# dleeim/Safe-Bayesian-Optimization

Hardware: AMD Instinct MI355X
Metric: candidate-points/sec, SafeOpt posterior+safe-set sweep (higher is better)
Workload: dtype f64

## Files before the change

include/safebo.h:

```cpp
#ifndef SAFEBO_H
#define SAFEBO_H

#include <stdint.h>

#ifdef __cplusplus
extern "C" {
#endif

#define SBO_ABI_VERSION 3
#define SBO_MAX_D 8
#define SBO_MAX_Q 8
#define SBO_MAX_N 2048

enum sbo_status {
  SBO_OK = 0,
  SBO_E_INVALID = -1,
  SBO_E_NOMEM = -2,
  SBO_E_HIP = -3,
  SBO_E_NO_MODEL = -4,
  SBO_E_NO_CANDIDATES = -5,
  SBO_E_EMPTY_SAFE_SET = -6,
  SBO_E_COMM = -7,
  SBO_E_UNSUPPORTED = -8
};
// ... 98 lines not shown
  double total_ms;
  double posterior_flops;
  int64_t candidates;
  int32_t posterior_launches;
  int32_t posterior_kernel;
  double posterior_executed_flops;
  double posterior_setup_ms;
  int64_t fp64_rechecks;
  double recheck_ms;
  double set_phase_ms;
  int32_t host_syncs;
  int32_t comm_calls;
  int64_t comm_bytes;
  double guard_dm[SBO_MAX_Q], guard_dv[SBO_MAX_Q], guard_rl[SBO_MAX_Q];
  double guard_ms;
  int32_t halo_reruns;
  int32_t set_path;
  int64_t guard_audit_samples, guard_audit_violations;
  double guard_audit_worst;
  double guard_analytic_dm[SBO_MAX_Q], guard_analytic_dv[SBO_MAX_Q], guard_probe_dm[SBO_MAX_Q], guard_probe_dv[SBO_MAX_Q];
  int64_t k1_tiles_skipped;
  int64_t k1_tiles_skipped_safe;
  int64_t k1_tiles_resident_c, k1_tiles_resident_o;
  int64_t guard_audit_skipped;
  double list_index_build_ms;
  int64_t list_index_leaf_pairs, list_index_nodes_skipped;
  double fp32_band_dm[SBO_MAX_Q], fp32_band_dv[SBO_MAX_Q];
} sbo_profile;

int sbo_version(void);
const char* sbo_last_error(void);
int sbo_device_count(int* count);
int sbo_init(int device_id, sbo_ctx** out);
int sbo_shutdown(sbo_ctx* ctx);
int sbo_synchronize(sbo_ctx* ctx);

#define SBO_COMM_ID_BYTES 128
int sbo_comm_unique_id(void* id_out );
int sbo_comm_init(sbo_ctx* ctx, int world_size, int rank, const void* id);
int sbo_comm_barrier(sbo_ctx* ctx);
typedef int (*sbo_relay_allreduce_fn)(void* user, void* buf, int64_t count, int elem, int op);
typedef int (*sbo_relay_allgather_fn)(void* user, const void* send, void* recv, int64_t bytes_per_rank);
int sbo_comm_init_relay(sbo_ctx* ctx, int world_size, int rank, sbo_relay_allreduce_fn allreduce,
                        sbo_relay_allgather_fn allgather, void* user);

int sbo_model_set(sbo_ctx* ctx, int dtype, const char* kernel, int n, int d, int q,
// ... 323 lines not shown
```

safe-bayesian-optimization_amd/_lib.py:

```python
from __future__ import annotations

import ctypes as C
import os

SBO_MAX_D = 8
SBO_MAX_Q = 8
SBO_MAX_N = 2048
SBO_COMM_ID_BYTES = 128
SBO_ROBUST_MAX_SCEN = 8
SBO_MAX_BATCH = 64
SBO_MAX_APPEND = 64
SBO_EXPANDER_MAX_POINTS = 65536
SBO_EXPANDER_MAX_SCRATCH = 1 << 32
SBO_MAX_PATHS = 64
SBO_MAX_FEATURES = 8192
SBO_PATHS_MAX_POINTS = 1 << 24
SBO_PATHS_MAX_VALUES = 1 << 32
SBO_REFINE_PATHS_MAX_STARTS = 64
SBO_JOINT_MAX_POINTS = 2048

SBO_F64, SBO_F32 = 0, 1
SBO_MEAN, SBO_UCB, SBO_LCB, SBO_VAR = 0, 1, 2, 3
SBO_MASK_S, SBO_MASK_U, SBO_MASK_M, SBO_MASK_G, SBO_MASK_O = 0, 1, 2, 3, 4

# ... 157 lines not shown
class JointOpts(C.Structure):
    _fields_ = [("output", C.c_int32), ("n_draws", C.c_int32), ("noise", C.c_int32), ("maximize", C.c_int32), ("jitter", C.c_double)]


class JointResult(C.Structure):
    _fields_ = [("index", C.c_int64 * SBO_MAX_PATHS), ("value", C.c_double * SBO_MAX_PATHS), ("pivot_min", C.c_double),
                ("pivot_row", C.c_int64)]


class Profile(C.Structure):
    _fields_ = [
        ("posterior_ms", C.c_double), ("classify_ms", C.c_double), ("expander_ms", C.c_double),
        ("argreduce_ms", C.c_double), ("comm_ms", C.c_double), ("total_ms", C.c_double),
        ("posterior_flops", C.c_double), ("candidates", C.c_int64), ("posterior_launches", C.c_int32),
        ("posterior_kernel", C.c_int32), ("posterior_executed_flops", C.c_double), ("posterior_setup_ms", C.c_double),
        ("fp64_rechecks", C.c_int64), ("recheck_ms", C.c_double),
        ("set_phase_ms", C.c_double), ("host_syncs", C.c_int32), ("comm_calls", C.c_int32), ("comm_bytes", C.c_int64),
        ("guard_dm", C.c_double * SBO_MAX_Q), ("guard_dv", C.c_double * SBO_MAX_Q), ("guard_rl", C.c_double * SBO_MAX_Q),
        ("guard_ms", C.c_double), ("halo_reruns", C.c_int32), ("set_path", C.c_int32),
        ("guard_audit_samples", C.c_int64), ("guard_audit_violations", C.c_int64), ("guard_audit_worst", C.c_double),
        ("guard_analytic_dm", C.c_double * SBO_MAX_Q), ("guard_analytic_dv", C.c_double * SBO_MAX_Q),
        ("guard_probe_dm", C.c_double * SBO_MAX_Q), ("guard_probe_dv", C.c_double * SBO_MAX_Q),
        ("k1_tiles_skipped", C.c_int64), ("k1_tiles_skipped_safe", C.c_int64),
        ("k1_tiles_resident_c", C.c_int64), ("k1_tiles_resident_o", C.c_int64), ("guard_audit_skipped", C.c_int64),
        ("list_index_build_ms", C.c_double), ("list_index_leaf_pairs", C.c_int64), ("list_index_nodes_skipped", C.c_int64),
        ("fp32_band_dm", C.c_double * SBO_MAX_Q), ("fp32_band_dv", C.c_double * SBO_MAX_Q),
    ]


RELAY_ALLREDUCE = C.CFUNCTYPE(C.c_int, C.c_void_p, C.c_void_p, C.c_int64, C.c_int, C.c_int)
RELAY_ALLGATHER = C.CFUNCTYPE(C.c_int, C.c_void_p, C.c_void_p, C.c_void_p, C.c_int64)

_P = C.c_void_p
_DP = C.POINTER(C.c_double)
SYMBOLS = [
    ("sbo_version", C.c_int, []),
    ("sbo_last_error", C.c_char_p, []),
    ("sbo_device_count", C.c_int, [C.POINTER(C.c_int)]),
    ("sbo_init", C.c_int, [C.c_int, C.POINTER(_P)]),
    ("sbo_shutdown", C.c_int, [_P]),
    ("sbo_synchronize", C.c_int, [_P]),
    ("sbo_comm_unique_id", C.c_int, [_P]),
    ("sbo_comm_init", C.c_int, [_P, C.c_int, C.c_int, _P]),
    ("sbo_comm_barrier", C.c_int, [_P]),
    ("sbo_comm_init_relay", C.c_int, [_P, C.c_int, C.c_int, RELAY_ALLREDUCE, RELAY_ALLGATHER, _P]),
    ("sbo_model_set", C.c_int, [_P, C.c_int, C.c_char_p, C.c_int, C.c_int, C.c_int, _P, _P, _P, _P, _P, _P, _P, _P]),
    ("sbo_model_set_list", C.c_int, [_P, C.c_int, C.c_char_p, C.c_int, C.c_int, C.c_int, _P, _P, _P, _P, _P, _P, _P, _P]),
# ... 92 lines not shown
```

safe-bayesian-optimization_amd/csrc/api.hip:

```cpp
#include <algorithm>
#include <cmath>
#include <cstring>
#include <limits>
#include <memory>
#include <chrono>
#include "internal.hpp"
#include "device_common.hpp"

namespace sbo {

static thread_local std::string g_err;

int fail(int code, const std::string& msg) {
  g_err = msg;
  return code;
}
int hip_fail(hipError_t e, const char* what) {
  g_err = std::string("HIP: ") + hipGetErrorString(e) + " in " + what;
  return SBO_E_HIP;
}
int ensure(DevBuf& b, size_t bytes) {
  if (bytes == 0) bytes = 16;
  if (b.bytes >= bytes) return SBO_OK;
  b.reset();
// ... 232 lines not shown
#define OPT_SCALED(key, field, scale, lo, hi, msg, effect, hook) {key, nullptr, &Options::field, kTakeScaled, msg, lo, hi, 0, scale, effect, hook}
const OptRow kOptions[] = {
    OPT_BOOL(halo_spec, kOptNothing, hook_halo),
    OPT_BOOL(comm_events, kOptNothing, nullptr),
    OPT_SCALED("cheb_tol_e17", cheb_tol, 1e-17, 0, 0, nullptr, kOptPlans, nullptr),
    OPT_RANGE(tensor_guess_pct, 10, 400, "tensor_guess_pct must be within 10 .. 400", kOptTensor, hook_tensor_guess),
    OPT_BOOL(tensor_cheb, kOptTensor, nullptr),
    OPT_CLAMP(exact_lazy, 0, 2, 1, kOptNothing, nullptr),
    OPT_BOOL(chol_async, kOptNothing, nullptr),
    OPT_RANGE(bilinear, 0, 2, "bilinear must be 0 (off), 1 (on; a model's first sweep by node interpolation) or 2 (on, K1b's plan from the first sweep)", kOptPlans, nullptr),
    OPT_BOOL(phase_events, kOptNothing, nullptr),
    OPT_RAW(scan_waves, kOptNothing, nullptr),
    OPT_BOOL(set_lanes, kOptNothing, nullptr),
    OPT_BOOL(result_mirror, kOptNothing, nullptr),
    OPT_BOOL(set_fuse, kOptNothing, nullptr),
    OPT_RANGE(col_path, 0, 2, "col_path must be 0 (never), 1 (auto) or 2 (whenever the grid's shape allows)", kOptNothing, nullptr),
    OPT_RANGE(guard_audit, 0, 1 << 20, "guard_audit: samples per sweep, 0 (off) .. 1048576", kOptNothing, hook_audit),
    OPT_SCALED("guard_audit_scale_ppm", audit_scale, 1e-6, 1, 1000000000, "guard_audit_scale_ppm: 1 .. 1e9", kOptNothing, hook_audit_scale),
    OPT_RANGE(guard_audit_every, 1, 1 << 20, "guard_audit_every: 1 .. 1048576 sweeps", kOptNothing, hook_audit_every),
    OPT_RANGE(grad_defer, 0, 3, "grad_defer must be 0 .. 3", kOptInterp, nullptr),
    OPT_BOOL(k1_sched, kOptNothing, nullptr),
    OPT_BOOL(k1_resident, kOptNothing, nullptr),
    OPT_BOOL(k1_skip_safe, kOptNothing, nullptr),
    OPT_BOOL(col_overlap, kOptNothing, nullptr),
    OPT_RANGE(col_queue, 64, 128, "col_queue must be within 64 .. 128 (the default)", kOptNothing, nullptr),
    OPT_BOOL(scan_blocks, kOptNothing, nullptr),
    OPT_RANGE(fuse_classify, -1, 1, "fuse_classify must be -1 (auto), 0 or 1", kOptNothing, nullptr),
    OPT_BOOL(goose_pairs, kOptNothing, nullptr),
    OPT_RANGE(guard_band, 0, 2, "guard_band must be 0 (off), 1 (on) or 2 (re-evaluate on every sweep)", kOptPlansBand, nullptr),
    OPT_BOOL(fp64_recheck, kOptNothing, nullptr),
    OPT_BOOL(comm_selftest, kOptNothing, hook_selftest),
    OPT_RANGE(refine_lds, 0, 1, "refine_lds must be 0 (stream M) or 1 (LDS when it fits)", kOptNothing, nullptr),
    OPT_RANGE(lipschitz_lds, 0, 1, "lipschitz_lds must be 0 (stream X_norm and alpha) or 1 (LDS when they fit)", kOptNothing, nullptr),
    OPT_RANGE(list_index, -1, 1, "list_index must be -1 (auto), 0 (never) or 1 (always)", kOptNothing, nullptr),
    OPT_RANGE(posterior_path, 0, 2, "posterior_path must be 0 (auto), 1 (generic) or 2 (generic, chunked)", kOptPosterior, nullptr),
};
#undef OPT_BOOL
#undef OPT_RANGE
#undef OPT_CLAMP
#undef OPT_RAW
#undef OPT_SCALED
}

int sbo_set_option(sbo_ctx* c, const char* key, int64_t value) {
  if (!c || !key) return fail(SBO_E_INVALID, "ctx/key is NULL");
  for (const OptRow& r : kOptions) {
// ... 494 lines not shown
```

safe-bayesian-optimization_amd/csrc/bilinear_post.inc.hpp:

```cpp


constexpr int kFuseRow = 4 + 2 * kMaxQ;
constexpr int kFuseVmin = 4, kFuseRmax = 4 + kMaxQ;
struct PostCtx {
  double* lds;
  int tid, lane, wave, rb0, cs0, nrb, ncs;
  int st_rb, st_cs, st_off, a_lo, b_st, a_rd;
  unsigned int ucnt0;
  long long nlines;
  bool full;
  bool imode;
  const double* var_rd;
  uint8_t *S, *U;
  double bconf, bb;
  int cS, cU;
  double rmax;
  LcbBand lband;
  bool gb_on;
  double vminS;
  int cB;
  int role;
  unsigned int bw[8];
  unsigned int* lds_bits;
  double umin;
// ... 1013 lines not shown
  const double gmax = ROLE == 1 ? lrec[ctile] : 0.0;
  post_partials<4>(sh, cx.lane, cx.wave, gmax, ROLE == 1, cx.cS, cx.cU, ROLE == 2 ? -cx.umin : cx.rmax, cx.cB, cx.vminS,
                   Lpart + ((size_t)o * tgy + by) * tgx + bx, cpart + (ROLE == 2 ? ntile : (size_t)0) + ctile, pcap, ROLE == 2, px.cb.slots,
                   (int)(ctile & (kColSlots - 1)), o, ROLE == 1 ? (int)by : -1, (int)bx, cx.xmin, false);
  if (ROLE == 1 && cx.tid < 128) {
    unsigned long long sw = 0ull, uw = 0ull;
#pragma unroll
    for (int w = 0; w < 4; ++w) {
      const unsigned int pc = bits[w * 128 + cx.tid];
      sw |= (unsigned long long)(pc & 0xffffu) << (16 * w);
      uw |= (unsigned long long)(pc >> 16) << (16 * w);
    }
    const size_t col = (size_t)cx.cs0 * 16u + cx.tid;
    px.cb.Sw[(size_t)by * cx.ucnt0 + col] = sw;
    px.cb.Uw[(size_t)by * cx.ucnt0 + col] = uw;
    if (uw != 0ull) atomicOr(&px.cb.Usum[col], 1ull << by);
  }
#ifdef SBO_PHASE_CLOCKS
  __syncthreads();
  if (threadIdx.x == 0) wg_trace_row(o, clk_in_, clk_ld_, wall_clock64(), (unsigned int)ctile, 4u);
#endif
}


__global__ __launch_bounds__(256, 3) void k_bgrad(const ModelConst mc, const CandSpec cs, const double* __restrict__ VA, size_t sVA,
                                                  const double* __restrict__ P0f, int KB, int nrb, int ncs, long long nlines, int gx, int gy,
                                                  const int* __restrict__ eff, const double* __restrict__ gtmax,
                                                  const unsigned long long* __restrict__ gkey, const double* __restrict__ xn0, int q,
                                                  double* __restrict__ Lpart, unsigned long long* __restrict__ slots,
                                                  int o_first ) {
  extern __shared__ double lds[];
  PostCtx cx;
  cx.lds = lds;
  cx.tid = threadIdx.x; cx.lane = cx.tid & 63; cx.wave = cx.tid >> 6;
  cx.nrb = nrb; cx.ncs = ncs;
  cx.ucnt0 = (unsigned int)cs.count[0];
  cx.nlines = nlines;
  cx.imode = true;
  const int st_i = cx.tid >> 5, st_j = cx.tid & 31;
  cx.st_off = st_j * 8;
  cx.a_lo = st_i < 4 ? st_i * 256 + (st_j >> 3) * 64 + (st_j & 7) * 4 : -1;
  cx.b_st = 1024 + st_i * 256 + cx.st_off;
  cx.a_rd = (((cx.lane >> 4) << 2) + (cx.lane & 3)) * 2;
  cx.var_rd = nullptr; cx.S = nullptr; cx.U = nullptr;
  cx.bconf = 0.0; cx.bb = 0.0; cx.cS = cx.cU = cx.cB = 0; cx.rmax = -1.0;
  cx.lband = LcbBand{0.0, 0.0}; cx.gb_on = false; cx.vminS = 1e300;
// ... 229 lines not shown
  SBO_HIP(hipFuncSetAttribute(reinterpret_cast<const void*>(k_bgrad), hipFuncAttributeMaxDynamicSharedMemorySize, (int)L.lds));
  hipLaunchKernelGGL(k_bgrad, dim3((unsigned)std::min<long long>((long long)L.rows_out, 2ll * c->n_cu)), dim3(256), L.lds, gs, c->mc, c->cs, g.VA,
                     g.sVA, g.P0f, g.KB0, g.nrb, g.ncs0, L.nlines, (int)L.gx, (int)L.gy, (const int*)g.eff, g.gtmax, g.gkey,
                     (const double*)c->bl_small.p, L.q, L.lrows, L.colw ? L.px.cb.slots : (unsigned long long*)nullptr, (L.req.sweep_lean && L.q >= 2) ? 1 : 0);
  SBO_HIP(hipEventRecord(c->ev_grad[2], gs));
  c->grad_pending = true;
  L.px.nograd = 1;
  return SBO_OK;
}

static void gemm_post_part(GemmLaunch& L, int part) {
  sbo_ctx* c = L.c;
  const GemmOps& g = L.g;
  const CandSpec& cs = c->cs;
  const bool colw = L.colw, fuse = L.fuse;
  const int q = L.q;
  const ColPartRows& rows = L.out.col_rows;
  PostExtra& px = L.px;
  px.o0 = colw ? 1 - part : 0;
  const bool last = !colw || part == 1;
  const decltype(&k_bpost<1, 0>) kposts[3] = {k_bpost<1, 0>, k_bpost<1, 1>, k_bpost<1, 2>};
  const auto kpost = kposts[colw ? 1 + part : 0];
  px.tlist = nullptr;
  if (L.sched_l1 && part == 0 && px.encl) {
    hipLaunchKernelGGL(k_bl_sched_tiles1, dim3((L.gx * L.gy + kSchedWaves - 1) / kSchedWaves), dim3(64 * kSchedWaves), 0, c->stream, c->mc, (const double*)px.encl, (int)(L.gx * L.gy), (int)L.gx,
                       (int)L.gy, (unsigned int)L.cnt0, L.req.fuse_b, L.gb_fused, g.gtmax, g.gkey, q, px.skip, L.sched_l1, L.sched_cap1, px.cb.Sw, px.cb.Uw,
                       px.cb.Usum, px.cb.slots, L.lrows, rows.base, rows.cap, px.skip_safe, L.res_rows ? (const double*)L.lrec : (const double*)nullptr,
                       L.res_c ? 1 : 0);
    px.tlist = L.sched_l1;
    px.tshift = kTlistShift;
    px.tcap = L.sched_cap1;
  }
  if (L.sched_l2 && part == 1) {
    hipLaunchKernelGGL(k_bl_sched_list2, dim3(1), dim3(1024), 0, c->stream, rows.base, rows.cap, (int)(L.gx * L.gy), L.sched_l2,
                       L.lrows, L.sched_l1, L.res_o ? (const uint8_t*)L.omap : (const uint8_t*)nullptr, px.cb.slots);
    px.tlist = L.sched_l2;
    px.tshift = 0;
    px.tcap = (int)(L.gx * L.gy);
    L.out.col_sched = true;
  }
  px.tgx = (int)L.gx;
  px.tgy = (int)L.gy;
  const dim3 grid = px.tlist ? dim3((unsigned)px.tcap << px.tshift) : dim3(L.gx, L.gy, (unsigned)(colw ? 1 : q));
  px.front_only = 0;
  const bool light_c = L.res_c && part == 0 && px.tlist != nullptr, light_o = L.res_o && part == 1 && px.tlist != nullptr;
  if (light_c) {
    hipExtLaunchKernelGGL(k_bres<1>, grid, dim3(256), 0, c->stream, nullptr, c->col.ev[0], 0, cs, (const double*)c->mean.p, (const double*)c->var.p,
                          L.lrows, L.req.fuse_b, (unsigned long long*)c->cpart.p, c->cpart_cap, L.gb_fused, (const double*)L.lrec, px);
  }
  if (light_o) {
    hipLaunchKernelGGL(k_bres<2>, grid, dim3(256), 0, c->stream, cs, (const double*)c->mean.p, (const double*)c->var.p, L.lrows, L.req.fuse_b,
                       (unsigned long long*)c->cpart.p, c->cpart_cap, (const GuardBand*)nullptr, (const double*)nullptr, px);
    px.front_only = 1;
  }
  if (!light_c) {
    hipExtLaunchKernelGGL(kpost, grid, dim3(256), L.lds, c->stream, nullptr,
                          (L.req.lmax_defer && last) ? c->ev[1] : ((colw && part == 0) ? c->col.ev[0] : nullptr), 0,
                          c->mc, cs, g.BtA, g.sBtA, g.P0f, g.sP0f, g.VA, g.sVA, g.SBf, g.sSBf, g.KB0, g.KS0, g.KBm, g.KSm, g.KBm2, g.nrb, g.ncs0,
                          L.nlines, (double*)c->mean.p, (double*)c->var.p, L.defer ? L.lrows + (size_t)L.rows_out * q : L.lrows,
                          (const double*)c->bl_small.p , fuse ? (uint8_t*)(q > 2 ? c->fuseS.p : c->maskS.p) : (uint8_t*)nullptr,
                          fuse ? (uint8_t*)(q > 2 ? c->fuseU.p : c->maskU.p) : (uint8_t*)nullptr, L.req.fuse_b, (unsigned long long*)c->cpart.p,
                          c->cpart_cap, L.gb_fused, (const int*)g.eff, g.gtmax, g.gkey, g.imode, px);
  }
  if (colw && part == 0 && L.record_encl) {
    hipLaunchKernelGGL(k_bl_enclose, dim3(L.gx, L.gy), dim3(128), 0, c->stream, (const double*)c->mean.p + (size_t)cs.n_local,
                       (const double*)c->var.p + (size_t)cs.n_local, L.cnt0, L.encl, (const double*)L.lrows + L.ntiles, L.lrec);
    c->bl.encl_ready = true;
    c->bl.lrows_ready = L.lrec != nullptr;
  }
  if (colw && part == 0 && !L.interp && c->bl.encl_ready && !px.encl) c->bl.vals_ready = true;
}

static void gemm_flops(const GemmLaunch& L) {
  sbo_ctx* c = L.c;
  const GemmOps& g = L.g;
  const int q = L.q;
  const double tiles2 = (double)g.nrb * g.ncs0;
  if (L.interp) {
// ... 68 lines not shown
```

safe-bayesian-optimization_amd/csrc/internal.hpp:

```cpp
#pragma once
#include <hip/hip_runtime.h>
#include <stddef.h>
#include <stdint.h>
#include <cmath>
#include <string>
#include <type_traits>
#include <vector>
#include "../../include/safebo.h"

namespace sbo {

constexpr int kGuardRefMaxNpad = 1008;
constexpr int kMaxD = SBO_MAX_D;
constexpr int kMaxQ = SBO_MAX_Q;

struct RcScal {
  unsigned long long ulo_key, uhi_key, vmax_key;
  long long count;
};
struct RcHead {
  RcScal sc;
  unsigned long long deferred;
  unsigned long long lmin_key;
  unsigned long long all_ranks;
// ... 108 lines not shown
  long long n = 0;
  int d = 0;
  int perm_half = 0;
  DevBuf box;
  DevBuf keys, vals, hist;
  DevBuf xs;
  DevBuf stats;
  Event ev0, ev1;
};

struct ColBits {
  unsigned long long* Sw;
  unsigned long long* Uw;
  unsigned long long* Usum;
  unsigned long long* slots;
};
constexpr int kColSlots = 64;
enum ColSlotField { kSlotUmin = 0 , kSlotS, kSlotU, kSlotB , kSlotVmin0, kSlotVmin1 ,
                    kSlotRmax1 , kSlotL0, kSlotL1 ,
                    kSlotRowMask ,
                    kSlotSkip ,
                    kSlotSkipSafe ,
                    kSlotResC, kSlotResO ,
                    kColSlotFields };
__host__ __device__ inline bool col_slot_is_min(int f) { return f == kSlotUmin || f == kSlotVmin0 || f == kSlotVmin1; }
constexpr unsigned int kTlistUnsafe = 0x80000000u, kTlistSafe = 0x40000000u;
constexpr unsigned char kSkipUnsafe = 1, kSkipSafe = 2;
constexpr int kTlistShift = 5, kTlistShards = 1 << kTlistShift, kTlistHead = 32;
struct PostExtra {
  int o0;
  int q;
  int lean;
  long long fstride;
  int nograd;
  ColBits cb;
  const double* encl;
  uint8_t* skip;
  int skip_safe;
  const unsigned int* tlist;
  int tshift, tcap;
  int tgx, tgy;
  int front_only;
  uint8_t* omap;
};

struct GemmOps {
// ... 216 lines not shown
  hipStream_t stream2 = nullptr;
  hipStream_t stream_audit = nullptr;
  hipStream_t stream4 = nullptr;
  hipStream_t stream3 = nullptr;
  int n_cu = 256;
  int decide_wg_per_cu = 1;
  struct Options {
    int chol_async = 1;
    int exact_lazy = 1;
    double cheb_tol = 4e-15;
    int tensor_cheb = 1;
    int tensor_guess_pct = 100;
    int guard_band = 1;
    int guard_audit = 1024;
    int guard_audit_every = 16;
    double audit_scale = 1.0;
    int set_lanes = 1;
    int refine_lds = 1;
    int lipschitz_lds = 1;
    int list_index = -1;
    int k1_sched = 1;
    int k1_resident = 1;
    int k1_skip_safe = 1;
    int comm_events = 0;
    int col_path = 1;
    int col_overlap = 1;
    int col_queue = 128;
    int grad_defer = 1;
    int halo_spec = 1;
    int scan_waves = 1;
    int scan_blocks = 1;
    int result_mirror = 1;
    int set_fuse = 1;
    int fuse_classify = -1;
    int goose_pairs = 0;
    int phase_events = 0;
    int bilinear = 1;
    int posterior_path = 0;
    int fp64_recheck = 1;
    int comm_selftest = 0;
  } opt;
  bool has_model = false;
  int dtype = SBO_F64;
  sbo::ModelConst mc{};
  sbo::DevBuf Fpk;
  sbo::DevBuf As;
// ... 285 lines not shown
```

safe-bayesian-optimization_amd/csrc/sets.hip:

```cpp
#include <algorithm>
#include <cstdio>
#include <cstdlib>
#include <cmath>
#include <cstring>
#include <type_traits>
#include <hip/hip_ext.h>
#include "device_common.hpp"

namespace sbo {

int comm_allreduce_max_u64(sbo_ctx* c, unsigned long long* dev, int count);
int comm_allreduce_min_u64(sbo_ctx* c, unsigned long long* dev, int count);
int comm_allreduce_sum_f64(sbo_ctx* c, double* dev, int count);
int comm_allgather_bytes(sbo_ctx* c, const void* send, void* recv, size_t bytes_per_rank);

constexpr double kInfD = 1.0e300;
constexpr int kArgSlots = 16;

struct SweepScalars {
  unsigned long long ustar_key;
  unsigned long long rmax_key[kMaxQ];
  long long count_S, count_U, count_M;
  long long count_set[kMaxQ];
  long long n_amb, n_amb_total;
  long long n_scan;
  long long halo_short;
  double arg_val[kArgSlots];
  long long arg_idx[kArgSlots];
  double arg_d[kArgSlots];
  long long n_guard;
  long long guard_slot[kArgSlots];
  long long tiles_skipped;
  long long tiles_skipped_safe;
  long long tiles_resident_c, tiles_resident_o;
  unsigned long long ticket;
  long long n_guard_cls;
  long long guard_nb0;
  unsigned long long vmin_key[kMaxQ];
  double gb_du[kMaxQ];
  double gb_rl[kMaxQ];
  double arg_e1[kArgSlots], arg_e2[kArgSlots];
  long long arg_ei[kArgSlots];
};
constexpr size_t kScalHost = offsetof(SweepScalars, ticket);
static_assert(sizeof(SweepScalars) <= sizeof(ScalBlock::scalars) && sizeof(SweepScalars) <= sizeof(PinnedBack::scalars), "SweepScalars fits its region of the scalar block and of the pinned block");

struct Best {
  double v;
  long long i;
  double d;
  double e1, e2;
  long long ei;
};
template <bool MAX>
__host__ __device__ __forceinline__ Best best_none() { return Best{0.0, -1, 0.0, MAX ? -kInfD : kInfD, MAX ? -kInfD : kInfD, -1}; }

template <bool MAX>
// ... 1898 lines not shown
  hipExtLaunchKernelGGL(k_sweep_finals<true>, dim3((unsigned)q), dim3(256), 0, c->stream, nullptr, mirrored ? c->ev[4] : nullptr, 0,
                        (const unsigned char*)pbase, pstride, n > 0 ? nb : 0, sc,
                        lanes ? (const SweepScalars*)c->lane[1].scal.p : (const SweepScalars*)nullptr,
                        mirrored ? (unsigned char*)c->h_back : (unsigned char*)nullptr, c->Lmax, gb_of<T>(c, v) ? 1 : 0);
  SBO_HIP(hipGetLastError());
  if ((rc = sweep_exchange_back(c, h, AllMax().v, Lk, c->ev[4], mirrored))) return rc;
  if (lazy_exact && (h.n_amb > 0 || c->opt.exact_lazy == 2) && (rc = late_exact_pass<T>(c, o, v, nb, h, Lk, launch_exact_d<T>))) return rc;
  if (multi_rank(c)) {
    sbo_sweep_opts o2 = *o;
    SetView v2 = v;
    if (halo_rerun(c, h, Lk, o2, v2)) return sweep_safeopt_t<T>(c, &o2, v2, res);
  }
  }
  c->masks_valid = true;
  c->last_sweep = 1;
  if (getenv("SBO_DEBUG_SCAN")) fprintf(stderr, "[safebo] open candidates scanned (last constraint) %lld, exact rechecks %lld\n", h.n_scan, h.n_amb_total);

  if ((rc = sweep_profile(c, kSafeOpt, reuse))) return rc;
  c->prof.set_path = colpath ? 1 : 0;
  c->prof.k1_tiles_skipped = colpath ? h.tiles_skipped : 0;
  c->prof.k1_tiles_skipped_safe = colpath ? h.tiles_skipped_safe : 0;
  c->prof.k1_tiles_resident_c = colpath ? h.tiles_resident_c : 0;
  c->prof.k1_tiles_resident_o = colpath ? h.tiles_resident_o : 0;
  if (colpath && !reuse)
    c->last_k1_flops = std::max(0.0, c->last_k1_flops - (double)h.tiles_resident_c * c->last_k1_tile_flops[1] - (double)h.tiles_resident_o * c->last_k1_tile_flops[0]);

  memset(res, 0, sizeof(*res));
  res->count_S = h.count_S;
  res->count_U = h.count_U;
  res->count_M = h.count_M;
  res->n_exact_rechecks = h.n_amb_total;
  res->guard_band = h.n_guard;
  c->gb.first = h.n_guard;
  for (int i = 0; i < q; ++i) memcpy(&res->L[i], &Lk[i], 8);
  if (o->lean && q >= 2) res->L[0] = 0.0;
  res->minimizer_index = -1;
  res->expander_index = -1;
  for (int cc = 1; cc <= kMaxQ; ++cc) res->expander_index_c[cc - 1] = -1;
  if (h.count_S == 0) return fail(SBO_E_EMPTY_SAFE_SET, "safe set S_t is empty on this candidate set");
  res->u_star = ord_val(h.ustar_key);
  res->minimizer_index = h.arg_idx[0];
  res->minimizer_std = std::sqrt(h.arg_val[0]);
  coords_of(c, res->minimizer_index, res->minimizer_x);
  double best_std = 0.0;
  int best_c = 0;
  for (int cc = 1; cc < q; ++cc) {
// ... 573 lines not shown
```

safe-bayesian-optimization_amd/csrc/sets_colpath.inc.hpp:

```cpp
#pragma once

struct ColGeom {
  int W, H, NS, NB;
  int NBp;
  int CW, CH;
  int CNB, CNBp, CWp;
  int gxt;
  double h0, h1;
  double delta;
};
constexpr int kColBig = 1 << 20;

typedef unsigned short us2_t __attribute__((ext_vector_type(2)));
__device__ __forceinline__ void col_fine_item(long long item, const ColGeom gm, const ColBits cb, unsigned short* __restrict__ tile,
                                              unsigned short* __restrict__ img, unsigned short* __restrict__ bmin,
                                              unsigned long long* __restrict__ Mw, unsigned long long* __restrict__ Gw) {
  const int lane = threadIdx.x & 63;
  const int ncg = gm.W >> 6;
  const int s = (int)(item / ncg), cgp = (int)(item % ncg);
  const int i = cgp * 64 + lane;
  Mw[(size_t)s * gm.W + i] = 0ull;
  Gw[(size_t)s * gm.W + i] = 0ull;
  const unsigned long long m = cb.Uw[(size_t)s * gm.W + i];
  const unsigned long long us = cb.Usum[i];
// ... 119 lines not shown
  }
#pragma unroll
  for (int k = 0; k < 32; ++k) {
    us2_t v;
    v[0] = (unsigned short)(pk[k] & 0xffffu);
    v[1] = (unsigned short)(pk[k] >> 16);
#pragma unroll
    for (int o = 16; o > 0; o >>= 1) {
      const unsigned int y = (unsigned int)__shfl_xor((int)((unsigned int)v[0] | ((unsigned int)v[1] << 16)), o);
      us2_t w2;
      w2[0] = (unsigned short)(y & 0xffffu);
      w2[1] = (unsigned short)(y >> 16);
      v = __builtin_elementwise_min(v, w2);
    }
    if (cl == k) {
      cbmin[(size_t)(64 * Sg + 2 * k) * gm.CNBp + blk] = v[0];
      cbmin[(size_t)(64 * Sg + 2 * k + 1) * gm.CNBp + blk] = v[1];
    }
  }
}

__device__ __forceinline__ unsigned long long col_slot_reduce(const unsigned long long* __restrict__ slots, int field) {
  unsigned long long v = slots[(size_t)field * kColSlots + (threadIdx.x & 63)];
  const bool is_min = col_slot_is_min(field), is_sum = field == kSlotS || field == kSlotU || field == kSlotB || field == kSlotSkip || field == kSlotSkipSafe || field == kSlotResC || field == kSlotResO;
#pragma unroll
  for (int o = 32; o > 0; o >>= 1) {
    const unsigned long long y = __shfl_xor(v, o);
    v = is_sum ? v + y : (is_min ? (y < v ? y : v) : (y > v ? y : v));
  }
  return v;
}
__device__ __forceinline__ void col_merge1_body(const unsigned long long* __restrict__ slots, SweepScalars* sc, unsigned long long* Lmax,
                                                const GuardBand* gb, double b) {
  unsigned long long* w = reinterpret_cast<unsigned long long*>(sc);
  for (unsigned i = threadIdx.x; i < sizeof(SweepScalars) / 8; i += blockDim.x) w[i] = 0ull;
  __syncthreads();
  if (threadIdx.x < 64) {
    const unsigned long long cS = col_slot_reduce(slots, kSlotS), cU = col_slot_reduce(slots, kSlotU), cB = col_slot_reduce(slots, kSlotB);
    const unsigned long long vmin = col_slot_reduce(slots, kSlotVmin1), rmax = col_slot_reduce(slots, kSlotRmax1), l1 = col_slot_reduce(slots, kSlotL1);
    const unsigned long long nskip = col_slot_reduce(slots, kSlotSkip), nsafe = col_slot_reduce(slots, kSlotSkipSafe), nresc = col_slot_reduce(slots, kSlotResC);
    if (threadIdx.x == 0) {
      Lmax[1] = l1;
      sc->tiles_skipped = (long long)nskip;
      sc->tiles_skipped_safe = (long long)nsafe;
      sc->tiles_resident_c = (long long)nresc;
      sc->ustar_key = ~0ull;
      sc->count_S = (long long)cS;
      sc->count_U = (long long)cU;
      sc->rmax_key[1] = rmax;
      if (gb) {
        sc->n_guard = (long long)cB;
        sc->n_guard_cls = (long long)cB;
        sc->vmin_key[1] = vmin;
        const bool any = vmin != ~0ull;
        const double vm = any ? fmax(0.0, ord_val(vmin)) : 0.0;
        sc->gb_du[1] = gb->dm[1] + (any ? b * gb_dsqrt(vm, gb->dv[1]) : 0.0);
        sc->gb_rl[0] = gb->rl[0];
        sc->gb_rl[1] = gb->rl[1];
      }
    }
  }
  if (threadIdx.x >= 64 && threadIdx.x < 64 + kArgSlots) sc->arg_idx[threadIdx.x - 64] = -1;
}
struct ColScal2 {
  unsigned long long ustar_key, vmin0_key;
  double gb_du0;
  unsigned long long res_o;
};
// ... 633 lines not shown
    else sc->count_set[slot - 1] += cnt;
    SweepScalars* hm = reinterpret_cast<SweepScalars*>(mirror);
    hm->arg_val[slot] = best.v;
    hm->arg_idx[slot] = best.i;
    hm->arg_d[slot] = best.d;
    hm->guard_slot[slot] = sc->guard_slot[slot];
    if (slot == 0) {
      hm->count_M = sc->count_M;
      sc->ustar_key = sc2->ustar_key;
      hm->ustar_key = sc2->ustar_key;
      hm->tiles_resident_o = (long long)sc2->res_o;
      for (int t = 2; t < kArgSlots; ++t) hm->guard_slot[t] = 0;
    } else {
      hm->count_set[slot - 1] = sc->count_set[slot - 1];
      hm->count_S = sc->count_S;
      hm->count_U = sc->count_U;
      hm->n_amb = sc->n_amb;
      hm->n_amb_total = sc->n_amb_total;
      hm->n_scan = sc->n_scan;
      hm->n_guard = sc->n_guard;
      hm->tiles_skipped = sc->tiles_skipped;
      hm->tiles_skipped_safe = sc->tiles_skipped_safe;
      hm->tiles_resident_c = sc->tiles_resident_c;
      for (int t = 0; t < kMaxQ; ++t) {
        hm->rmax_key[t] = sc->rmax_key[t];
        reinterpret_cast<unsigned long long*>(mirror + offsetof(PinnedBack, lip_keys))[t] = Lkeys[t];
      }
    }
  }
}

__global__ __launch_bounds__(256) void k_col_expand(const unsigned long long* __restrict__ Wd, int W, long long n, uint8_t* __restrict__ out) {
  for (long long g = (long long)blockIdx.x * blockDim.x + threadIdx.x; g < n; g += (long long)gridDim.x * blockDim.x) {
    const long long j = g / W;
    const int i = (int)(g - j * W);
    out[g] = (uint8_t)((Wd[(size_t)(j >> 6) * W + i] >> (j & 63)) & 1ull);
  }
}
static void col_expand(sbo_ctx* c, const DevBuf& words, uint8_t* out) {
  const long long n = c->cs.n_local;
  hipLaunchKernelGGL(k_col_expand, dim3((unsigned)std::min<long long>((n + 255) / 256, 1 << 16)), dim3(256), 0, c->stream,
                     (const unsigned long long*)words.p, (int)c->cs.count[0], n, out);
}

int col_decide_resident(int* wg_per_cu) {
  SBO_HIP(hipOccupancyMaxActiveBlocksPerMultiprocessor(wg_per_cu, k_col_decide, 256, 0));
// ... 200 lines not shown
```

Baseline: 83.35 billion.

## Add fused head kernel classifying only undecided cells of mixed K1 tiles

Result: faster. 90.99 billion (median of 6 runs) (+9.2%).

```diff
diff --git a/include/safebo.h b/include/safebo.h
--- a/include/safebo.h
+++ b/include/safebo.h
@@ -144,6 +144,7 @@
   int64_t k1_tiles_skipped;
   int64_t k1_tiles_skipped_safe;
   int64_t k1_tiles_resident_c, k1_tiles_resident_o;
+  int64_t k1_cells_evaluated;
   int64_t guard_audit_skipped;
   double list_index_build_ms;
   int64_t list_index_leaf_pairs, list_index_nodes_skipped;
diff --git a/safe-bayesian-optimization_amd/_lib.py b/safe-bayesian-optimization_amd/_lib.py
--- a/safe-bayesian-optimization_amd/_lib.py
+++ b/safe-bayesian-optimization_amd/_lib.py
@@ -203,7 +203,8 @@
         ("guard_analytic_dm", C.c_double * SBO_MAX_Q), ("guard_analytic_dv", C.c_double * SBO_MAX_Q),
         ("guard_probe_dm", C.c_double * SBO_MAX_Q), ("guard_probe_dv", C.c_double * SBO_MAX_Q),
         ("k1_tiles_skipped", C.c_int64), ("k1_tiles_skipped_safe", C.c_int64),
-        ("k1_tiles_resident_c", C.c_int64), ("k1_tiles_resident_o", C.c_int64), ("guard_audit_skipped", C.c_int64),
+        ("k1_tiles_resident_c", C.c_int64), ("k1_tiles_resident_o", C.c_int64), ("k1_cells_evaluated", C.c_int64),
+        ("guard_audit_skipped", C.c_int64),
         ("list_index_build_ms", C.c_double), ("list_index_leaf_pairs", C.c_int64), ("list_index_nodes_skipped", C.c_int64),
         ("fp32_band_dm", C.c_double * SBO_MAX_Q), ("fp32_band_dv", C.c_double * SBO_MAX_Q),
     ]
diff --git a/safe-bayesian-optimization_amd/csrc/api.hip b/safe-bayesian-optimization_amd/csrc/api.hip
--- a/safe-bayesian-optimization_amd/csrc/api.hip
+++ b/safe-bayesian-optimization_amd/csrc/api.hip
@@ -278,6 +278,7 @@
     OPT_BOOL(k1_sched, kOptNothing, nullptr),
     OPT_BOOL(k1_resident, kOptNothing, nullptr),
     OPT_BOOL(k1_skip_safe, kOptNothing, nullptr),
+    OPT_BOOL(k1_cells, kOptNothing, nullptr),
     OPT_BOOL(col_overlap, kOptNothing, nullptr),
     OPT_RANGE(col_queue, 64, 128, "col_queue must be within 64 .. 128 (the default)", kOptNothing, nullptr),
     OPT_BOOL(scan_blocks, kOptNothing, nullptr),
diff --git a/safe-bayesian-optimization_amd/csrc/bilinear_post.inc.hpp b/safe-bayesian-optimization_amd/csrc/bilinear_post.inc.hpp
--- a/safe-bayesian-optimization_amd/csrc/bilinear_post.inc.hpp
+++ b/safe-bayesian-optimization_amd/csrc/bilinear_post.inc.hpp
@@ -1059,6 +1059,307 @@
 #endif
 }
 
+struct CandAcc { double vminS, xmin, rmax; };
+__device__ __forceinline__ void post_classify_cand(double m, double v, double bconf, double bb, bool gb_on, const LcbBand& lband, bool& ge_out,
+                                                   bool& le_out, bool& near_out, CandAcc& a) {
+  constexpr double c = 1.0 + 0x1p-48, tiny = 1e-250, huge = 1e300;
+  const bool bok = bconf >= 0.0;
+  const double P = m * m, Q = bb * v;
+  near_out = false;
+  if (gb_on) {
+    const double gap = P > Q ? P - Q : Q - P, am = m < 0 ? -m : m;
+    near_out = !(gap > fma(am, lband.c1, lband.c0));
+  }
+  const bool ok = bok && v >= 0.0, rng = P < huge && Q < huge;
+  const bool neg = ok && m < 0.0;
+  bool ge = ok && !neg && rng && P > tiny && P >= Q * c;
+  bool le = neg || (ok && rng && !ge && Q > tiny && P * c <= Q && m >= 0.0);
+  if (!ge && !le) {
+    const double sd = mul_rn(bconf, sqrt_rn(v));
+    ge = m >= sd;
+    le = m <= sd;
+  }
+  if (ge) {
+    a.vminS = v < a.vminS ? v : a.vminS;
+    const float sf = __builtin_amdgcn_sqrtf((float)v);
+    const double s_up = (double)sf * (1.0 + 0x1p-20) + 1e-18;
+    double s_lo = (double)sf * (1.0 - 0x1p-20) - 1e-18;
+    s_lo = s_lo > 0.0 ? s_lo : 0.0;
+    const bool fin = sf < 3.0e38f;
+    const double xu = m + bconf * s_up, xl = m + bconf * (fin ? s_lo : 0.0);
+    const double up = fin ? xu + (xu < 0 ? -xu : xu) * 0x1p-50 : 1e300, lo = xl - (xl < 0 ? -xl : xl) * 0x1p-50;
+    a.xmin = lo < a.xmin ? lo : a.xmin;
+    if (!(up <= a.rmax)) {
+      const double ucb = add_rn(m, mul_rn(bconf, sqrt_rn(v)));
+      if (ucb > a.rmax) a.rmax = ucb;
+    }
+  }
+  ge_out = ge;
+  le_out = le;
+}
+
+constexpr int kHeadWaves = 4, kHeadBatch = 4;
+struct HeadRec { unsigned int cS, cU, cB, ncell; unsigned long long vmin, rmax, xmin; };
+__global__ __launch_bounds__(64 * kHeadWaves) void k_bhead(const double* __restrict__ encl, int ntiles, int tgx, int tgy, unsigned int cnt0, double bconf,
+                                                           const GuardBand* __restrict__ gb, const double* __restrict__ mean1,
+                                                           const double* __restrict__ var1 ,
+                                                           uint8_t* __restrict__ skip, unsigned long long* __restrict__ Sw,
+                                                           unsigned long long* __restrict__ Uw, unsigned long long* __restrict__ Usum,
+                                                           unsigned long long* __restrict__ slots, double* __restrict__ Lpart,
+                                                           unsigned long long* __restrict__ cpart, int pcap, int skip_safe,
+                                                           const double* __restrict__ lrec) {
+  __shared__ unsigned long long sh_w[kHeadWaves][2][128];
+  __shared__ unsigned short sh_q[kHeadWaves * 128];
+  __shared__ HeadRec sh_rec[kHeadWaves];
+  __shared__ unsigned int sh_xy[kHeadWaves];
+  __shared__ unsigned int sh_qn;
+  __shared__ unsigned long long sh_acc[kHeadWaves][10];
+  const int lane = threadIdx.x & 63, wave = (int)(threadIdx.x >> 6);
+  const unsigned long long below = (1ull << lane) - 1ull;
+  const double bb = bconf * bconf;
+  const bool gb_on = gb != nullptr;
+  const LcbBand lb = gb_on ? lcb_band(bb, gb->dm[1], gb->dv[1]) : LcbBand{0.0, 0.0};
+  unsigned long long a_key = 0ull, a_vmin = ~0ull, a_rmax = 0ull;
+  unsigned int a_S = 0u, a_U = 0u, a_B = 0u, a_n0 = 0u, a_n4 = 0u, a_res = 0u, a_cells = 0u;
+#ifdef SBO_PHASE_CLOCKS
+  const unsigned long long clk_in_ = wall_clock64();
+  unsigned long long clk_dec_ = clk_in_;
+  unsigned int clk_tile_ = 0xffffffu;
+#endif
+  const int per_round = kHeadWaves * (int)gridDim.x;
+  for (int t0 = 0; t0 < ntiles; t0 += per_round) {
+    const int tile = t0 + wave * (int)gridDim.x + (int)blockIdx.x;
+    const bool have = tile < ntiles;
+    if (threadIdx.x == 0) sh_qn = 0u;
+    __syncthreads();
+    bool mixed = false;
+    int bx = 0, by = 0;
+    double lrow = 0.0;
+    if (have) {
+      bx = tile % tgx;
+      by = tile / tgx;
+      lrow = lrec[tile];
+      a_key = (unsigned long long)__double_as_longlong(lrow) > a_key ? (unsigned long long)__double_as_longlong(lrow) : a_key;
+      bool us[2], sf[2];
+      double kv = 1e300, ku = -1.0, kl = 1e300;
+#pragma unroll
+      for (int h = 0; h < 2; ++h) {
+        const double4 e = reinterpret_cast<const double4*>(encl)[(size_t)tile * 128 + h * 64 + lane];
+        us[h] = encl_unsafe(e.x, e.y, e.z, e.w, bconf, bb, gb_on, lb);
+        sf[h] = skip_safe != 0 && !us[h] && encl_safe(e.x, e.y, e.z, e.w, bconf, bb, gb_on, lb);
+        if (sf[h]) {
+          const EnclKeys ek = encl_keys(e.x, e.y, e.z, e.w, bconf);
+          kv = ek.vlo < kv ? ek.vlo : kv;
+          ku = ek.up > ku ? ek.up : ku;
+          kl = ek.lo < kl ? ek.lo : kl;
+        }
+      }
+      const unsigned long long mU[2] = {__ballot(us[0]), __ballot(us[1])}, mS[2] = {__ballot(sf[0]), __ballot(sf[1])};
+      const bool dec = (mU[0] & mU[1]) == ~0ull, sdec = (mS[0] & mS[1]) == ~0ull;
+      const size_t w0 = (size_t)by * cnt0 + (size_t)bx * 128;
+      if (lane == 0) {
+        skip[tile] = dec ? kSkipUnsafe : (sdec ? kSkipSafe : 0);
+        Lpart[((size_t)tgy + by) * tgx + bx] = lrow;
+      }
+      if (!dec) {
+#pragma unroll
+        for (int off = 32; off > 0; off >>= 1) {
+          const double ov = __shfl_xor(kv, off), ou = __shfl_xor(ku, off), ol = __shfl_xor(kl, off);
+          kv = ov < kv ? ov : kv;
+          ku = ou > ku ? ou : ku;
+          kl = ol < kl ? ol : kl;
+        }
+      }
+      const unsigned long long kvmin = kv < 1e300 ? ord_key(kv) : ~0ull, krmax = ku >= 0.0 ? ord_key(ku) : 0ull, kxmin = kl < 1e300 ? ord_key(kl) : ~0ull;
+      if (dec) {
+#pragma unroll
+        for (int h = 0; h < 2; ++h) {
+          Sw[w0 + h * 64 + lane] = 0ull;
+          Uw[w0 + h * 64 + lane] = ~0ull;
+          atomicOr(&Usum[(size_t)bx * 128 + h * 64 + lane], 1ull << by);
+        }
+        if (lane < kFuseRow) {
+          unsigned long long v = 0ull;
+          if (lane == 0) v = ~0ull;
+          else if (lane == 2) v = 64ull * 128ull;
+          else if (lane >= kFuseVmin && lane < kFuseRmax) v = ~0ull;
+          cpart[(size_t)lane * pcap + tile] = v;
+        }
+        a_n0 += 1u;
+      } else if (sdec) {
+#pragma unroll
+        for (int h = 0; h < 2; ++h) {
+          Sw[w0 + h * 64 + lane] = ~0ull;
+          Uw[w0 + h * 64 + lane] = 0ull;
+        }
+        if (lane == 0) atomicOr(&slots[(size_t)kSlotRowMask * kColSlots + by], 1ull << bx);
+        if (lane < kFuseRow) {
+          unsigned long long v = 0ull;
+          if (lane == 0) v = kxmin;
+          else if (lane == 1) v = 64ull * 128ull;
+          else if (lane >= kFuseVmin && lane < kFuseRmax) v = lane == kFuseVmin + 1 ? kvmin : ~0ull;
+          else if (lane == kFuseRmax + 1) v = krmax;
+          cpart[(size_t)lane * pcap + tile] = v;
+        }
+        a_n4 += 1u;
+        a_vmin = kvmin < a_vmin ? kvmin : a_vmin;
+        a_rmax = krmax > a_rmax ? krmax : a_rmax;
+      } else {
+        mixed = true;
+#pragma unroll
+        for (int h = 0; h < 2; ++h) {
+          const int cc = (h * 64 + lane) >> 3;
+          unsigned long long sw = 0ull, uw = 0ull;
+#pragma unroll
+          for (int cr = 0; cr < 8; ++cr) {
+            const int bit = 16 * (cr & 3) + cc;
+            sw |= ((mS[cr >> 2] >> bit) & 1ull) ? 0xffull << (8 * cr) : 0ull;
+            uw |= ((mU[cr >> 2] >> bit) & 1ull) ? 0xffull << (8 * cr) : 0ull;
+          }
+          sh_w[wave][0][h * 64 + lane] = sw;
+          sh_w[wave][1][h * 64 + lane] = uw;
+        }
+        const unsigned long long mN[2] = {~(mU[0] | mS[0]), ~(mU[1] | mS[1])};
+        const unsigned int n0 = (unsigned int)__popcll(mN[0]), n1 = (unsigned int)__popcll(mN[1]);
+        unsigned int base = 0u;
+        if (lane == 0) {
+          base = atomicAdd(&sh_qn, n0 + n1);
+          sh_rec[wave] = HeadRec{64u * (unsigned int)(__popcll(mS[0]) + __popcll(mS[1])), 64u * (unsigned int)(__popcll(mU[0]) + __popcll(mU[1])), 0u,
+                                 n0 + n1, kvmin, krmax, kxmin};
+          sh_xy[wave] = (unsigned int)bx | ((unsigned int)by << 16);
+        }
+        base = (unsigned int)__shfl((int)base, 0);
+        if ((mN[0] >> lane) & 1ull) sh_q[base + (unsigned int)__popcll(mN[0] & below)] = (unsigned short)((wave << 7) | lane);
+        if ((mN[1] >> lane) & 1ull) sh_q[base + n0 + (unsigned int)__popcll(mN[1] & below)] = (unsigned short)((wave << 7) | (64 + lane));
+      }
+    }
+    __syncthreads();
+#ifdef SBO_PHASE_CLOCKS
+    if (t0 == 0) clk_dec_ = wall_clock64();
+    if (mixed && clk_tile_ == 0xffffffu) clk_tile_ = (unsigned int)tile;
+#endif
+    {
+      const unsigned int nq = sh_qn;
+      const unsigned int r8 = (unsigned int)lane & 7u, c8 = (unsigned int)lane >> 3;
+      CandAcc acc{1e300, 1e300, -1.0};
+      unsigned int cS = 0u, cU = 0u, cB = 0u;
+      int cur = -1;
+      auto flush = [&]() {
+        if (cur < 0) return;
+        double vm = acc.vminS, xm = acc.xmin, rm = acc.rmax;
+#pragma unroll
+        for (int off = 32; off > 0; off >>= 1) {
+          const double ov = __shfl_xor(vm, off), ox = __shfl_xor(xm, off), orr = __shfl_xor(rm, off);
+          vm = ov < vm ? ov : vm;
+          xm = ox < xm ? ox : xm;
+          rm = orr > rm ? orr : rm;
+        }
+        if (lane == 0) {
+          HeadRec& r = sh_rec[cur];
+          if (cS) atomicAdd(&r.cS, cS);
+          if (cU) atomicAdd(&r.cU, cU);
+          if (cB) atomicAdd(&r.cB, cB);
+          if (vm < 1e300) atomicMin(&r.vmin, ord_key(vm));
+          if (xm < 1e300) atomicMin(&r.xmin, ord_key(xm));
+          if (rm >= 0.0) atomicMax(&r.rmax, ord_key(rm));
+        }
+        acc = CandAcc{1e300, 1e300, -1.0};
+        cS = cU = cB = 0u;
+      };
+      for (unsigned int b0 = (unsigned int)wave * kHeadBatch; b0 < nq; b0 += kHeadWaves * kHeadBatch) {
+        unsigned int ent[kHeadBatch];
+        double m[kHeadBatch], v[kHeadBatch];
+#pragma unroll
+        for (int k = 0; k < kHeadBatch; ++k) {
+          ent[k] = (unsigned int)__builtin_amdgcn_readfirstlane((int)sh_q[b0 + k < nq ? b0 + k : b0]);
+          const unsigned int xy = (unsigned int)__builtin_amdgcn_readfirstlane((int)sh_xy[ent[k] >> 7]), cell = ent[k] & 127u;
+          const size_t g = ((size_t)(xy >> 16) * 64 + (size_t)(cell >> 4) * 8 + r8) * cnt0 + (size_t)(xy & 0xffffu) * 128 + (size_t)(cell & 15u) * 8 + c8;
+          m[k] = mean1[g];
+          v[k] = var1[g];
+        }
+#pragma unroll
+        for (int k = 0; k < kHeadBatch; ++k) {
+          if (b0 + k < nq) {
+            const int w = (int)(ent[k] >> 7);
+            const unsigned int cell = ent[k] & 127u;
+            if (w != cur) {
+              flush();
+              cur = w;
+            }
+            bool ge, le, nr;
+            post_classify_cand(m[k], v[k], bconf, bb, gb_on, lb, ge, le, nr, acc);
+            const unsigned long long gm = __ballot(ge), lm = __ballot(le);
+            cS += (unsigned int)__popcll(gm);
+            cU += (unsigned int)__popcll(lm);
+            cB += (unsigned int)__popcll(__ballot(nr));
+            if (lane < 16) {
+              const unsigned long long bits = lane < 8 ? gm : lm;
+              reinterpret_cast<unsigned char*>(&sh_w[w][lane >> 3][(cell & 15u) * 8 + (lane & 7)])[cell >> 4] = (unsigned char)(bits >> (8 * (lane & 7)));
+            }
+          }
+        }
+      }
+      flush();
+    }
+    __syncthreads();
+    if (mixed) {
+      const size_t w0 = (size_t)by * cnt0 + (size_t)bx * 128;
+#pragma unroll
+      for (int h = 0; h < 2; ++h) {
+        const unsigned long long sw = sh_w[wave][0][h * 64 + lane], uw = sh_w[wave][1][h * 64 + lane];
+        Sw[w0 + h * 64 + lane] = sw;
+        Uw[w0 + h * 64 + lane] = uw;
+        if (uw != 0ull) atomicOr(&Usum[(size_t)bx * 128 + h * 64 + lane], 1ull << by);
+      }
+      const HeadRec r = sh_rec[wave];
+      if (lane == 0 && r.cS != 0u) atomicOr(&slots[(size_t)kSlotRowMask * kColSlots + by], 1ull << bx);
+      if (lane < kFuseRow) {
+        unsigned long long v = 0ull;
+        if (lane == 0) v = r.xmin;
+        else if (lane == 1) v = r.cS;
+        else if (lane == 2) v = r.cU;
+        else if (lane == 3) v = r.cB;
+        else if (lane >= kFuseVmin && lane < kFuseRmax) v = lane == kFuseVmin + 1 ? r.vmin : ~0ull;
+        else if (lane == kFuseRmax + 1) v = r.rmax;
+        cpart[(size_t)lane * pcap + tile] = v;
+      }
+      a_S += r.cS;
+      a_U += r.cU;
+      a_B += r.cB;
+      a_res += 1u;
+      a_cells += r.ncell;
+      a_vmin = r.vmin < a_vmin ? r.vmin : a_vmin;
+      a_rmax = r.rmax > a_rmax ? r.rmax : a_rmax;
+    }
+  }
+  if (lane == 0) {
+    unsigned long long* a = sh_acc[wave];
+    a[0] = a_key; a[1] = (unsigned long long)a_S + 64ull * 128ull * a_n4; a[2] = (unsigned long long)a_U + 64ull * 128ull * a_n0; a[3] = a_B; a[4] = a_n0; a[5] = a_n4;
+    a[6] = a_res; a[7] = a_cells;
+    a[8] = a_vmin; a[9] = a_rmax;
+  }
+  __syncthreads();
+  if (threadIdx.x < 10) {
+    const int f = (int)threadIdx.x;
+    unsigned long long x = sh_acc[0][f];
+#pragma unroll
+    for (int w = 1; w < kHeadWaves; ++w) {
+      const unsigned long long y = sh_acc[w][f];
+      x = f == 8 ? (y < x ? y : x) : ((f == 0 || f == 9) ? (y > x ? y : x) : x + y);
+    }
+    const int slot = (int)(blockIdx.x & (kColSlots - 1));
+    const int field = f == 0 ? kSlotL1 : f == 1 ? kSlotS : f == 2 ? kSlotU : f == 3 ? kSlotB : f == 4 ? kSlotSkip : f == 5 ? kSlotSkipSafe :
+                      f == 6 ? kSlotResC : f == 7 ? kSlotCells : f == 8 ? kSlotVmin1 : kSlotRmax1;
+    unsigned long long* p = &slots[(size_t)field * kColSlots + slot];
+    if (f == 8) { if (x != ~0ull) atomicMin(p, x); }
+    else if (f == 0 || f == 9) { if (x != 0ull) atomicMax(p, x); }
+    else if (x != 0ull) atomicAdd(p, x);
+  }
+#ifdef SBO_PHASE_CLOCKS
+  if (threadIdx.x == 0) wg_trace_row(1, clk_in_, clk_dec_, wall_clock64(), clk_tile_, 5u);
+#endif
+}
+
 
 __global__ __launch_bounds__(256, 3) void k_bgrad(const ModelConst mc, const CandSpec cs, const double* __restrict__ VA, size_t sVA,
                                                   const double* __restrict__ P0f, int KB, int nrb, int ncs, long long nlines, int gx, int gy,
@@ -1334,7 +1635,16 @@
   const decltype(&k_bpost<1, 0>) kposts[3] = {k_bpost<1, 0>, k_bpost<1, 1>, k_bpost<1, 2>};
   const auto kpost = kposts[colw ? 1 + part : 0];
   px.tlist = nullptr;
-  if (L.sched_l1 && part == 0 && px.encl) {
+  const bool head_c = L.res_c && c->opt.k1_cells && L.sched_l1 && part == 0 && px.encl;
+  if (head_c) {
+    const unsigned nt = L.gx * L.gy;
+    const unsigned hgrid = std::max(1u, std::min((nt + kHeadWaves - 1) / kHeadWaves, 4u * (unsigned)c->n_cu));
+    hipExtLaunchKernelGGL(k_bhead, dim3(hgrid), dim3(64 * kHeadWaves), 0, c->stream, nullptr, c->col.ev[0], 0, (const double*)px.encl, (int)nt, (int)L.gx,
+                          (int)L.gy, (unsigned int)L.cnt0, L.req.fuse_b, L.gb_fused, (const double*)c->mean.p + (size_t)cs.n_local,
+                          (const double*)c->var.p + (size_t)cs.n_local, px.skip, px.cb.Sw, px.cb.Uw, px.cb.Usum, px.cb.slots, L.lrows, rows.base,
+                          rows.cap, px.skip_safe, (const double*)L.lrec);
+  }
+  if (L.sched_l1 && part == 0 && px.encl && !head_c) {
     hipLaunchKernelGGL(k_bl_sched_tiles1, dim3((L.gx * L.gy + kSchedWaves - 1) / kSchedWaves), dim3(64 * kSchedWaves), 0, c->stream, c->mc, (const double*)px.encl, (int)(L.gx * L.gy), (int)L.gx,
                        (int)L.gy, (unsigned int)L.cnt0, L.req.fuse_b, L.gb_fused, g.gtmax, g.gkey, q, px.skip, L.sched_l1, L.sched_cap1, px.cb.Sw, px.cb.Uw,
                        px.cb.Usum, px.cb.slots, L.lrows, rows.base, rows.cap, px.skip_safe, L.res_rows ? (const double*)L.lrec : (const double*)nullptr,
@@ -1365,7 +1675,7 @@
                        (unsigned long long*)c->cpart.p, c->cpart_cap, (const GuardBand*)nullptr, (const double*)nullptr, px);
     px.front_only = 1;
   }
-  if (!light_c) {
+  if (!light_c && !head_c) {
     hipExtLaunchKernelGGL(kpost, grid, dim3(256), L.lds, c->stream, nullptr,
                           (L.req.lmax_defer && last) ? c->ev[1] : ((colw && part == 0) ? c->col.ev[0] : nullptr), 0,
                           c->mc, cs, g.BtA, g.sBtA, g.P0f, g.sP0f, g.VA, g.sVA, g.SBf, g.sSBf, g.KB0, g.KS0, g.KBm, g.KSm, g.KBm2, g.nrb, g.ncs0,
diff --git a/safe-bayesian-optimization_amd/csrc/internal.hpp b/safe-bayesian-optimization_amd/csrc/internal.hpp
--- a/safe-bayesian-optimization_amd/csrc/internal.hpp
+++ b/safe-bayesian-optimization_amd/csrc/internal.hpp
@@ -154,6 +154,7 @@
                     kSlotSkip ,
                     kSlotSkipSafe ,
                     kSlotResC, kSlotResO ,
+                    kSlotCells ,
                     kColSlotFields };
 __host__ __device__ inline bool col_slot_is_min(int f) { return f == kSlotUmin || f == kSlotVmin0 || f == kSlotVmin1; }
 constexpr unsigned int kTlistUnsafe = 0x80000000u, kTlistSafe = 0x40000000u;
@@ -416,6 +417,7 @@
     int k1_sched = 1;
     int k1_resident = 1;
     int k1_skip_safe = 1;
+    int k1_cells = 1;
     int comm_events = 0;
     int col_path = 1;
     int col_overlap = 1;
diff --git a/safe-bayesian-optimization_amd/csrc/sets.hip b/safe-bayesian-optimization_amd/csrc/sets.hip
--- a/safe-bayesian-optimization_amd/csrc/sets.hip
+++ b/safe-bayesian-optimization_amd/csrc/sets.hip
@@ -33,6 +33,7 @@
   long long tiles_skipped;
   long long tiles_skipped_safe;
   long long tiles_resident_c, tiles_resident_o;
+  long long cells_evaluated;
   unsigned long long ticket;
   long long n_guard_cls;
   long long guard_nb0;
@@ -1977,6 +1978,7 @@
   c->prof.k1_tiles_skipped_safe = colpath ? h.tiles_skipped_safe : 0;
   c->prof.k1_tiles_resident_c = colpath ? h.tiles_resident_c : 0;
   c->prof.k1_tiles_resident_o = colpath ? h.tiles_resident_o : 0;
+  c->prof.k1_cells_evaluated = colpath ? h.cells_evaluated : 0;
   if (colpath && !reuse)
     c->last_k1_flops = std::max(0.0, c->last_k1_flops - (double)h.tiles_resident_c * c->last_k1_tile_flops[1] - (double)h.tiles_resident_o * c->last_k1_tile_flops[0]);
 
diff --git a/safe-bayesian-optimization_amd/csrc/sets_colpath.inc.hpp b/safe-bayesian-optimization_amd/csrc/sets_colpath.inc.hpp
--- a/safe-bayesian-optimization_amd/csrc/sets_colpath.inc.hpp
+++ b/safe-bayesian-optimization_amd/csrc/sets_colpath.inc.hpp
@@ -165,7 +165,7 @@
 
 __device__ __forceinline__ unsigned long long col_slot_reduce(const unsigned long long* __restrict__ slots, int field) {
   unsigned long long v = slots[(size_t)field * kColSlots + (threadIdx.x & 63)];
-  const bool is_min = col_slot_is_min(field), is_sum = field == kSlotS || field == kSlotU || field == kSlotB || field == kSlotSkip || field == kSlotSkipSafe || field == kSlotResC || field == kSlotResO;
+  const bool is_min = col_slot_is_min(field), is_sum = field == kSlotS || field == kSlotU || field == kSlotB || field == kSlotSkip || field == kSlotSkipSafe || field == kSlotResC || field == kSlotResO || field == kSlotCells;
 #pragma unroll
   for (int o = 32; o > 0; o >>= 1) {
     const unsigned long long y = __shfl_xor(v, o);
@@ -181,12 +181,13 @@
   if (threadIdx.x < 64) {
     const unsigned long long cS = col_slot_reduce(slots, kSlotS), cU = col_slot_reduce(slots, kSlotU), cB = col_slot_reduce(slots, kSlotB);
     const unsigned long long vmin = col_slot_reduce(slots, kSlotVmin1), rmax = col_slot_reduce(slots, kSlotRmax1), l1 = col_slot_reduce(slots, kSlotL1);
-    const unsigned long long nskip = col_slot_reduce(slots, kSlotSkip), nsafe = col_slot_reduce(slots, kSlotSkipSafe), nresc = col_slot_reduce(slots, kSlotResC);
+    const unsigned long long nskip = col_slot_reduce(slots, kSlotSkip), nsafe = col_slot_reduce(slots, kSlotSkipSafe), nresc = col_slot_reduce(slots, kSlotResC), ncells = col_slot_reduce(slots, kSlotCells);
     if (threadIdx.x == 0) {
       Lmax[1] = l1;
       sc->tiles_skipped = (long long)nskip;
       sc->tiles_skipped_safe = (long long)nsafe;
       sc->tiles_resident_c = (long long)nresc;
+      sc->cells_evaluated = (long long)ncells;
       sc->ustar_key = ~0ull;
       sc->count_S = (long long)cS;
       sc->count_U = (long long)cU;
@@ -866,6 +867,7 @@
       hm->tiles_skipped = sc->tiles_skipped;
       hm->tiles_skipped_safe = sc->tiles_skipped_safe;
       hm->tiles_resident_c = sc->tiles_resident_c;
+      hm->cells_evaluated = sc->cells_evaluated;
       for (int t = 0; t < kMaxQ; ++t) {
         hm->rmax_key[t] = sc->rmax_key[t];
         reinterpret_cast<unsigned long long*>(mirror + offsetof(PinnedBack, lip_keys))[t] = Lkeys[t];
```
